# bootphon/abnet3

Hardware: AMD Instinct MI355X
Metric: frame-pairs/sec (Siamese train step: fwd both towers + coscos2 + bwd + Adadelta) (higher is better)
Workload: dtype f16x2; 1 GPU; C2: SiameseNetwork 40->500x2->100 sigmoid, coscos2(avg=False), Adadelta(0.1), 4096 frame pairs per GPU per step, 40-d N(0,1) frames; pairs_per_gpu=4096, global_pairs=4096, parallelism=dp1, graph_replay=False, dp_gradient_buckets=1

## Files before the change

### abnet3_amd/csrc/common.h

```cpp
#pragma once
#include <hip/hip_runtime.h>
#include <stdint.h>
#include <stdio.h>

#include "../../include/abnet3_hip.h"

namespace abn {

void set_error(const char* fmt, ...);

#define ABN_REQUIRE(cond, ...)                      \
    do {                                            \
        if (!(cond)) {                              \
            ::abn::set_error(__VA_ARGS__);          \
            return ABN_E_ARG;                       \
        }                                           \
    } while (0)

#define ABN_CHECK_LAUNCH(what)                                               \
    do {                                                                     \
        hipError_t e_ = hipGetLastError();                                   \
        if (e_ != hipSuccess) {                                              \
            ::abn::set_error("%s: %s", what, hipGetErrorString(e_));         \
            return ABN_E_LAUNCH;                                             \
        }                                                                    \
    } while (0)

struct Switches {
    bool planes;
    bool fused;
    int64_t fused_min_rows;
    bool bn_planes;
    bool bn_persist;
    bool wgrad_xcd;
    bool bf16x3_planes;
    bool bwd_pair;
    int gemm_tile;
    bool dtw_f40, dtw_pc;
    int wgrad_tile128;
    int dtw_wgs_per_cu;
    int wgrad_wgs_heavy, wgrad_wgs_light;
    int64_t wgrad_rows_per_slab;
    bool wide;
    int64_t wide_max_rows;
    int wide_max_groups;
    bool wgrad_step;
    bool dtw_dealt;
    int oneshot_wgs;
    int knn_split;
    int sd_tiles;
};
const Switches& switches();
void reload_switches();

__device__ __forceinline__ bool abn_ticket_publish(double* slot, double value, unsigned* counter, unsigned n_tickets)
{
    __hip_atomic_store(slot, value, __ATOMIC_RELAXED, __HIP_MEMORY_SCOPE_AGENT);
#ifdef ABN_STRICT_FENCES
    const unsigned ticket = __hip_atomic_fetch_add(counter, 1u, __ATOMIC_ACQ_REL, __HIP_MEMORY_SCOPE_AGENT);
#else
    __atomic_signal_fence(__ATOMIC_SEQ_CST);
    __builtin_amdgcn_s_waitcnt(0);
    __atomic_signal_fence(__ATOMIC_SEQ_CST);
    const unsigned ticket = __hip_atomic_fetch_add(counter, 1u, __ATOMIC_RELAXED, __HIP_MEMORY_SCOPE_AGENT);
#endif
    return ticket == n_tickets - 1;
}
__device__ __forceinline__ double abn_ticket_partial(const double* slot)
{
    return __hip_atomic_load(slot, __ATOMIC_RELAXED, __HIP_MEMORY_SCOPE_AGENT);
}

static inline int64_t align_up(int64_t v, int64_t a) { return (v + a - 1) / a * a; }
static inline bool aligned16(const void* p) { return (reinterpret_cast<uintptr_t>(p) & 15) == 0; }

static inline int device_slot()
{
    int dev = 0;
    (void)hipGetDevice(&dev);
    return (dev >= 0 && dev < 16) ? dev : 0;
}
static inline bool first_use_on_device(bool (&seen)[16])
{
    bool& s = seen[device_slot()];
    const bool first = !s;
    s = true;
    return first;
}

}
```

### abnet3_amd/csrc/tower_planes.h

```cpp
#pragma once
#include <type_traits>

#include "gemm_f32.h"

namespace abn {

typedef int v4i __attribute__((ext_vector_type(4)));

constexpr int PL_ROWS = 32;
constexpr int PL_WAVES = 8;
constexpr int PL_NT = 64 * PL_WAVES;
constexpr int PL_MAXW = 512;
constexpr int PL_MAXSTEPS = PL_MAXW / 16;
#ifdef PL_DEPTH_OVERRIDE
constexpr int PL_DEPTH = PL_DEPTH_OVERRIDE;
#else
constexpr int PL_DEPTH = 4;
#endif
constexpr int PL_PART_BYTES = 4 * 16 * 64 * 4;
constexpr int PL_SC_BYTES = PL_WAVES * 64 * 4 + PL_WAVES * 32 * 4;
constexpr int PL_AMAX = 32;

__host__ __device__ inline int pl_steps(int64_t contraction) { return ((int)((contraction + 15) / 16) + PL_DEPTH - 1) / PL_DEPTH * PL_DEPTH; }
__host__ __device__ inline int pl_blocks(int64_t features) { return (int)((features + 31) / 32); }
// ... 930 lines not shown
#pragma unroll
            for (int pl = 0; pl < NP; ++pl) *reinterpret_cast<bf16x8*>(img + ((int64_t)s * NP + pl) * 1024 + lane * 16) = z;
    }
    __syncthreads();
}

template <int NP, bool INFER>
__device__ __forceinline__ void planes_input_stage(const PlanesFwdP& p, char* __restrict__ img, float* __restrict__ part,
                                                   const bf16x8* idf, int wave, int lane, int row0, float& ainv, int row_end = -1)
{
    const int rows_lim = row_end >= 0 ? row_end : p.rows;
    const int r = lane & 31, h = lane >> 5;
    const int D0 = p.dims[0];
    const int steps0 = pl_steps(D0), blocks0 = steps0 / 2;
    const int gr = row0 + r;
    const float* src = nullptr;
    if (gr < rows_lim) src = (p.x2 && gr >= p.rows_call) ? p.x2 + (int64_t)(gr - p.rows_call) * D0 : p.x1 + (int64_t)gr * D0;
    float* const sc = part + PL_PART_BYTES / 4;
    const float* const inv_tab = sc + PL_WAVES * 64 + wave * 32;
    if constexpr (NP == 2) {
        f32x4 v[2][2][2];
        float m = 0.0f;
#pragma unroll
        for (int u = 0; u < 2; ++u) {
            const int kb = wave + PL_WAVES * u;
#pragma unroll
            for (int t2 = 0; t2 < 2; ++t2) {
                const int c0 = 16 * (2 * kb + t2) + 4 * h, c1 = c0 + 8;
                v[u][t2][0] = v[u][t2][1] = f32x4{0.f, 0.f, 0.f, 0.f};
                if (src && kb < blocks0 && c0 < D0) {
                    v[u][t2][0] = *reinterpret_cast<const f32x4*>(src + c0);
                    if (p.x_copy) *reinterpret_cast<f32x4*>(p.x_copy + (int64_t)gr * D0 + c0) = v[u][t2][0];
                }
                if (src && kb < blocks0 && c1 < D0) {
                    v[u][t2][1] = *reinterpret_cast<const f32x4*>(src + c1);
                    if (p.x_copy) *reinterpret_cast<f32x4*>(p.x_copy + (int64_t)gr * D0 + c1) = v[u][t2][1];
                }
                m = fmaxf(m, absmax8(v[u][t2][0], v[u][t2][1]));
            }
        }
        sc[wave * 64 + lane] = m;
        __syncthreads();
        float osc;
        m = row_scales(sc, wave, lane, osc, ainv);
        if (!INFER && p.tp[0] && wave == 0) store_amax_rows(p.amax[0] + (int64_t)blockIdx.x * PL_AMAX, m, 1.0f, lane);
#pragma unroll
        for (int u = 0; u < 2; ++u) {
            const int kb = wave + PL_WAVES * u;
            if (kb < blocks0) {
                Frag<NP> f[2];
#pragma unroll
                for (int t2 = 0; t2 < 2; ++t2) {
                    f[t2] = make_frag<NP>(v[u][t2][0], v[u][t2][1], osc);
                    store_frag<NP>(img + (int64_t)(2 * kb + t2) * (NP * 1024) + lane * 16, f[t2]);
                }
                if (!INFER && p.tp[0] && kb < pl_blocks(D0 + 1))
                    emit_planes<NP>(p.tp[0] + ((int64_t)kb * p.tp_steps + 2 * blockIdx.x) * tile_bytes<NP>(), f, idf, lane,
                                    kb == D0 / 32 ? D0 % 32 : -1, rows_lim - row0, inv_tab);
            }
        }
    } else {
        for (int kb = wave; kb < blocks0; kb += PL_WAVES) {
            Frag<NP> f[2];
#pragma unroll
            for (int t2 = 0; t2 < 2; ++t2) {
                const int s = 2 * kb + t2;
                f32x4 v0 = {0.f, 0.f, 0.f, 0.f}, v1 = v0;
                const int c0 = 16 * s + 4 * h, c1 = c0 + 8;
                if (src && c0 < D0) {
                    v0 = *reinterpret_cast<const f32x4*>(src + c0);
                    if (p.x_copy) *reinterpret_cast<f32x4*>(p.x_copy + (int64_t)gr * D0 + c0) = v0;
                }
                if (src && c1 < D0) {
                    v1 = *reinterpret_cast<const f32x4*>(src + c1);
                    if (p.x_copy) *reinterpret_cast<f32x4*>(p.x_copy + (int64_t)gr * D0 + c1) = v1;
                }
                f[t2] = make_frag<NP>(v0, v1);
                store_frag<NP>(img + (int64_t)s * (NP * 1024) + lane * 16, f[t2]);
            }
            if (!INFER && p.tp[0] && kb < pl_blocks(D0 + 1))
                emit_planes<NP>(p.tp[0] + ((int64_t)kb * p.tp_steps + 2 * blockIdx.x) * tile_bytes<NP>(), f, idf, lane,
                                kb == D0 / 32 ? D0 % 32 : -1, rows_lim - row0);
        }
    }
    if (!INFER && p.tp[0] && pl_blocks(D0 + 1) > blocks0 && wave == PL_WAVES - 1) {
        Frag<NP> z[2] = {};
        emit_planes<NP>(p.tp[0] + ((int64_t)(D0 / 32) * p.tp_steps + 2 * blockIdx.x) * tile_bytes<NP>(), z, idf, lane, 0, rows_lim - row0, inv_tab);
    }
}

template <int NP, int MODE = PL_TRAIN>
__global__ __launch_bounds__(PL_NT) void tower_fwd_planes_kernel(PlanesFwdP p)
{
    constexpr bool INFER = MODE != PL_TRAIN;
    extern __shared__ __attribute__((aligned(16))) char pl_smem[];
    char* const img = pl_smem;
    float* const part = reinterpret_cast<float*>(pl_smem + PL_MAXSTEPS * NP * 1024);
    const int lane = threadIdx.x & 63;
    const int wave = __builtin_amdgcn_readfirstlane(threadIdx.x >> 6);
    const int row0 = blockIdx.x * PL_ROWS;
    bf16x8 idf[2];
    make_identity<NP>(idf, lane);
    PSTAMPF(0);
#ifdef PL_EXP_PRIO
    if ((PL_EXP_PRIO == 1) == (wave >= 4)) __builtin_amdgcn_s_setprio(1);
#endif

    float ainv = 1.0f;
    WeightRing<NP> ring;
    ring_open(ring, p.wbase, p.wbytes);
    constexpr bool STAG = PL_STAGGER && NP <= 2 && (MODE == PL_TRAIN || MODE == PL_INFER);
    Stag st;
    if constexpr (STAG) stag_open(st, pl_smem, NP, threadIdx.x);
    planes_input_stage<NP, INFER>(p, img, part, idf, wave, lane, row0, ainv);
    PSTAMPF(1);
    __syncthreads();

    for (int l = 0; l < p.n_layers; ++l) {
        const int nblk = (p.dims[l + 1] + 31) / 32;
        if constexpr (STAG) {
            char* const cur = st.in();
            const bool out_halves = nblk > PL_WAVES && l + 1 < p.n_layers && (p.dims[l + 2] + 31) / 32 > PL_WAVES;
            if (nblk > PL_WAVES) planes_layer<NP, 2, 1, MODE>(p, l, cur, part, idf, wave, lane, row0, ainv, ring, -1, st, true, out_halves);
            else if (nblk > PL_WAVES / 2 || pl_steps(p.dims[l]) % (2 * PL_DEPTH) != 0) planes_layer<NP, 1, 1, MODE>(p, l, cur, part, idf, wave, lane, row0, ainv, ring);
            else planes_layer<NP, 1, 2, MODE>(p, l, cur, part, idf, wave, lane, row0, ainv, ring);
        } else {
            if (nblk > PL_WAVES) planes_layer<NP, 2, 1, MODE>(p, l, img, part, idf, wave, lane, row0, ainv, ring);
            else if (nblk > PL_WAVES / 2 || pl_steps(p.dims[l]) % (2 * PL_DEPTH) != 0) planes_layer<NP, 1, 1, MODE>(p, l, img, part, idf, wave, lane, row0, ainv, ring);
            else planes_layer<NP, 1, 2, MODE>(p, l, img, part, idf, wave, lane, row0, ainv, ring);
        }
    }
    PSTAMPF(2 + 5 * p.n_layers);
}

struct BnTrainP {
    int l;
    const float* mean;
    const float* invstd;
    const float* z_prev;
    float* a_prev;
    const int* n_valid;
};

template <int NP>
__global__ __launch_bounds__(PL_NT) void bn_fwd_layer_kernel(PlanesFwdP p, BnTrainP q)
{
    extern __shared__ __attribute__((aligned(16))) char pl_smem[];
    char* const img = pl_smem;
    float* const part = reinterpret_cast<float*>(pl_smem + PL_MAXSTEPS * NP * 1024);
    const int lane = threadIdx.x & 63;
    const int wave = __builtin_amdgcn_readfirstlane(threadIdx.x >> 6);
    const int r = lane & 31, h = lane >> 5;
    const int wpc = (p.rows_call + PL_ROWS - 1) / PL_ROWS;
    const int call = blockIdx.x / wpc;
    const int row0 = call * p.rows_call + (blockIdx.x - call * wpc) * PL_ROWS;
    const int row_end = call * p.rows_call + (q.n_valid ? min(max(*q.n_valid, 0), p.rows_call) : p.rows_call);
    const int l = q.l;
    bf16x8 idf[2];
    make_identity<NP>(idf, lane);
    float ainv = 1.0f;
    WeightRing<NP> ring;
    ring_open(ring, p.wbase, p.wbytes);

    if (l == 0) {
        planes_input_stage<NP, false>(p, img, part, idf, wave, lane, row0, ainv, row_end);
    } else {
        const int K = p.dims[l];
        float* const mean_s = part, * const is_s = part + PL_MAXW, * const ga_s = part + 2 * PL_MAXW, * const be_s = part + 3 * PL_MAXW;
        for (int c = threadIdx.x; c < K; c += PL_NT) {
            mean_s[c] = q.mean[(int64_t)call * K + c];
            is_s[c] = q.invstd[(int64_t)call * K + c];
            ga_s[c] = p.bn_w[l - 1][c];
            be_s[c] = p.bn_b[l - 1][c];
        }
        __syncthreads();
        const int steps = pl_steps(K), blocks = steps / 2;
        const int gr = row0 + r;
        const bool row_ok = gr < row_end;
        const float* const zrow = q.z_prev + (int64_t)(row_ok ? gr : row0) * K;
        float* const arow = q.a_prev ? q.a_prev + (int64_t)gr * K : nullptr;
        char* const tp = p.tp[l];
        float* const sc = part + PL_PART_BYTES / 4;
        const float* const inv_tab = sc + PL_WAVES * 64 + wave * 32;
        with_act(p.act[l - 1], [&](auto tag) {
            constexpr int ACT = decltype(tag)::value;
            auto in_step = [&](int s, f32x4* v) {
                v[0] = v[1] = f32x4{0.f, 0.f, 0.f, 0.f};
#pragma unroll
                for (int u = 0; u < 2; ++u) {
                    const int c = 16 * s + 4 * h + 8 * u;
                    if (c < K && row_ok) {
                        const f32x4 z4 = *reinterpret_cast<const f32x4*>(zrow + c);
                        const f32x4 mu = *reinterpret_cast<const f32x4*>(mean_s + c), is = *reinterpret_cast<const f32x4*>(is_s + c);
                        const f32x4 ga = *reinterpret_cast<const f32x4*>(ga_s + c), be = *reinterpret_cast<const f32x4*>(be_s + c);
#pragma unroll
                        for (int e = 0; e < 4; ++e) v[u][e] = act_apply(((z4[e] - mu[e]) * is[e]) * ga[e] + be[e], ACT);
                        if (arow) *reinterpret_cast<f32x4*>(arow + c) = v[u];
                    }
                }
            };
            if constexpr (NP == 2) {
                f32x4 v[2][2][2];
                float m = 0.0f;
#pragma unroll
                for (int u = 0; u < 2; ++u)
#pragma unroll
                    for (int t2 = 0; t2 < 2; ++t2) {
                        const int kb = wave + PL_WAVES * u;
                        v[u][t2][0] = v[u][t2][1] = f32x4{0.f, 0.f, 0.f, 0.f};
                        if (kb < blocks) in_step(2 * kb + t2, v[u][t2]);
                        m = fmaxf(m, absmax8(v[u][t2][0], v[u][t2][1]));
                    }
                sc[wave * 64 + lane] = m;
                __syncthreads();
                float osc;
                m = row_scales(sc, wave, lane, osc, ainv);
                if (tp && wave == 0) store_amax_rows(p.amax[l] + (int64_t)blockIdx.x * PL_AMAX, m, 1.0f, lane);
#pragma unroll
                for (int u = 0; u < 2; ++u) {
                    const int kb = wave + PL_WAVES * u;
                    if (kb < blocks) {
                        Frag<NP> f[2];
#pragma unroll
                        for (int t2 = 0; t2 < 2; ++t2) {
                            f[t2] = make_frag<NP>(v[u][t2][0], v[u][t2][1], osc);
                            store_frag<NP>(img + (int64_t)(2 * kb + t2) * (NP * 1024) + lane * 16, f[t2]);
                        }
                        if (tp && kb < pl_blocks(K + 1))
                            emit_planes<NP>(tp + ((int64_t)kb * p.tp_steps + 2 * blockIdx.x) * tile_bytes<NP>(), f, idf, lane,
                                            kb == K / 32 ? K % 32 : -1, row_end - row0, inv_tab);
                    }
                }
            } else {
                for (int kb = wave; kb < blocks; kb += PL_WAVES) {
                    Frag<NP> f[2];
#pragma unroll
                    for (int t2 = 0; t2 < 2; ++t2) {
                        f32x4 v[2];
                        in_step(2 * kb + t2, v);
                        f[t2] = make_frag<NP>(v[0], v[1]);
                        store_frag<NP>(img + (int64_t)(2 * kb + t2) * (NP * 1024) + lane * 16, f[t2]);
                    }
                    if (tp && kb < pl_blocks(K + 1))
                        emit_planes<NP>(tp + ((int64_t)kb * p.tp_steps + 2 * blockIdx.x) * tile_bytes<NP>(), f, idf, lane,
                                        kb == K / 32 ? K % 32 : -1, row_end - row0);
                }
            }
        });
        if (tp && pl_blocks(K + 1) > blocks && wave == PL_WAVES - 1) {
            Frag<NP> z[2] = {};
            emit_planes<NP>(tp + ((int64_t)(K / 32) * p.tp_steps + 2 * blockIdx.x) * tile_bytes<NP>(), z, idf, lane, 0, row_end - row0, inv_tab);
        }
    }
    __syncthreads();

    const int nblk = (p.dims[l + 1] + 31) / 32;
    if (nblk > PL_WAVES) planes_layer<NP, 2, 1, PL_BN_TRAIN>(p, l, img, part, idf, wave, lane, row0, ainv, ring, row_end);
    else if (nblk > PL_WAVES / 2 || pl_steps(p.dims[l]) % (2 * PL_DEPTH) != 0) planes_layer<NP, 1, 1, PL_BN_TRAIN>(p, l, img, part, idf, wave, lane, row0, ainv, ring, row_end);
    else planes_layer<NP, 1, 2, PL_BN_TRAIN>(p, l, img, part, idf, wave, lane, row0, ainv, ring, row_end);
}

struct PlanesBwdP {
    int n_layers;
    int rows;
    int dims[ABN_MAX_LAYERS + 1];
    int act[ABN_MAX_LAYERS];
    const float* d_out;
    int d_out_is_dz;
    const float* a_top;
    const char* tp[ABN_MAX_LAYERS];
    float* dx;
    const float* mask[ABN_MAX_LAYERS];
    const char* wpt[ABN_MAX_LAYERS];
    const char* wbase;
    int64_t wbytes;
    char* dzp[ABN_MAX_LAYERS];
    float* amax_dz[ABN_MAX_LAYERS];
    int64_t tp_steps;
    const unsigned long long* drop_seed;
    float drop_p;
    int loss_kind;
    int y_dtype;
    const void* y;
    int B;
    double margin, scale;
    double* loss_partial;
    unsigned* loss_counter;
    float* loss_out;
    const int* n_valid;
    double* loss_accum;
#ifdef ABN_STAMPS
    unsigned long long* stamps;
#endif
};
#ifdef ABN_STAMPS
#define DSTAMP(slot) do { if (p.stamps && threadIdx.x == 0) p.stamps[(size_t)blockIdx.x * 64 + (slot)] = __builtin_amdgcn_s_memtime(); } while (0)
#else
#define DSTAMP(slot) do {} while (0)
#endif

template <int NP, int BPW, int KS>
__device__ __forceinline__ void planes_dgrad_layer(const PlanesBwdP& p, int l, char* __restrict__ img,
                                                   float* __restrict__ part, const bf16x8* idf, int wave, int lane, int row0, float& ainv,
                                                   WeightRing<NP>& ring)
{
    const int N = p.dims[l + 1], K = p.dims[l];
    const int nsteps = pl_steps(N), nblk = (K + 31) / 32;
    const int r = lane & 31, h = lane >> 5;
    const WaveShare<BPW, KS> ws(wave, nblk, nsteps);
    const int blk0 = ws.blk0;

    f32x16 acc[BPW];
#pragma unroll
    for (int j = 0; j < BPW; ++j)
#pragma unroll
        for (int q = 0; q < 16; ++q) acc[j][q] = 0.0f;
    float cinv[BPW];
#pragma unroll
    for (int j = 0; j < BPW; ++j) cinv[j] = NP == 2 && ws.active ? packed_inv(p.wpt[l], nblk, nsteps, blk0 + j) * ainv : 1.0f;
    {
        bool chain_next = false;
        int nblk2 = 1, nsteps2 = 0, ioff2 = 0;
        if constexpr (PL_HANDOVER && NP <= 2 && BPW == 2 && KS == 1) {
            if (l - 1 >= (p.dx ? 0 : 1)) {
                nblk2 = (p.dims[l - 1] + 31) / 32;
                nsteps2 = pl_steps(K);
                ioff2 = (int)(p.wpt[l - 1] - p.wbase);
                chain_next = nblk2 > PL_WAVES;
            }
        }
        if (!ws.active) ring.filled = false;
        const int ioff = (int)(p.wpt[l] - p.wbase);
        int wv[BPW], dnext[BPW];
#pragma unroll
        for (int j = 0; j < BPW; ++j) {
            const int blk = blk0 + j < nblk ? blk0 + j : nblk - 1;
            const int o = ioff + (blk * nsteps + ws.s_first) * (NP * 1024);
            const int blk2 = blk0 + j < nblk2 ? blk0 + j : nblk2 - 1;
            wv[j] = o + lane * 16;
            dnext[j] = ioff2 + blk2 * nsteps2 * (NP * 1024) - o;
        }
        if (ws.active) ring_kloop<NP, BPW>(acc, ring, wv, dnext, chain_next, img, ws.s_first, ws.my_steps, lane);
    }
    DSTAMP(4 + 4 * (p.n_layers - 1 - l));

    const float* __restrict__ mask = l >= 1 ? p.mask[l - 1] : nullptr;
    const DropGen drop = make_drop(l >= 1 && !mask ? p.drop_seed : nullptr, p.drop_p, l - 1);
    const bool masked = mask || drop.on;
    const int gr = row0 + r;
    const bool row_ok = gr < p.rows;
    const int grc = row_ok ? gr : p.rows - 1;
    f32x4 av[BPW][4], mv[BPW][4];
    if (ws.active && ws.khalf == 0 && l >= 1) {
        const int row_off = tgather_row_offset<NP>(r);
#pragma unroll
        for (int j = 0; j < BPW; ++j) {
            const int blk = blk0 + j < nblk ? blk0 + j : nblk - 1;
            const char* tile = p.tp[l] + ((int64_t)blk * p.tp_steps + 2 * blockIdx.x) * tile_bytes<NP>();
#pragma unroll
            for (int g = 0; g < 4; ++g) {
#pragma unroll
                for (int e = 0; e < 4; ++e) av[j][g][e] = tgather<NP>(tile, row_off, 8 * g + 4 * h + e);
                const int k = 32 * (blk0 + j) + 4 * h + 8 * g;
                if (mask) mv[j][g] = *reinterpret_cast<const f32x4*>(mask + (int64_t)grc * K + (k < K ? k : K - 4));
                else if (drop.on) mv[j][g] = drop4(drop, gr, k);
            }
        }
    }
    auto finish = [&]() {
        if constexpr (NP == 2) {
#pragma unroll
            for (int j = 0; j < BPW; ++j)
#pragma unroll
                for (int q = 0; q < 16; ++q) acc[j][q] *= cinv[j];
        }
        if (l == 0) return;
        with_act(p.act[l - 1], [&](auto tag) {
            constexpr int ACT = decltype(tag)::value;
#pragma unroll
            for (int j = 0; j < BPW; ++j)
#pragma unroll
                for (int g = 0; g < 4; ++g) {
                    const bool live = 32 * (blk0 + j) + 4 * h + 8 * g < K;
#pragma unroll
                    for (int e = 0; e < 4; ++e) {
                        float v = acc[j][4 * g + e] * act_grad(av[j][g][e], ACT);
                        if (masked) v *= mv[j][g][e];
                        acc[j][4 * g + e] = live ? v : 0.0f;
                    }
                }
        });
    };
    float* const sc = part + PL_PART_BYTES / 4;
    const bool rescale = NP == 2 && l >= 1;
    auto park_max = [&]() {
        float m = 0.0f;
        if (ws.active && ws.khalf == 0) {
#pragma unroll
            for (int j = 0; j < BPW; ++j)
#pragma unroll
                for (int q = 0; q < 16; ++q) m = fmaxf(m, fabsf(acc[j][q]));
        }
        sc[wave * 64 + lane] = m;
    };
    if (KS == 1) {
        if (ws.active) finish();
        if (rescale) park_max();
    } else if (ws.active && ws.khalf == 1) {
#pragma unroll
        for (int q = 0; q < 16; ++q) part[((wave & 3) * 16 + q) * 64 + lane] = acc[0][q];
    }
    DSTAMP(5 + 4 * (p.n_layers - 1 - l));
    __syncthreads();
    DSTAMP(6 + 4 * (p.n_layers - 1 - l));
    if (KS == 2 && ws.active && ws.khalf == 0) {
#pragma unroll
        for (int q = 0; q < 16; ++q) acc[0][q] += part[(wave * 16 + q) * 64 + lane];
        finish();
    }
    float osc = 1.0f;
    if (rescale) {
        if (KS == 2) { park_max(); __syncthreads(); }
        float oinv;
        const float m = row_scales(sc, wave, lane, osc, oinv);
        ainv = oinv;
        if (wave == 0) store_amax_rows(p.amax_dz[l - 1] + (int64_t)blockIdx.x * PL_AMAX, m, 0.0f, lane);
    }
    const float* const inv_tab = sc + PL_WAVES * 64 + wave * 32;
    if (ws.active && ws.khalf == 0) {
#pragma unroll
        for (int j = 0; j < BPW; ++j) {
            const int blk = blk0 + j;
            if (blk < nblk) {
                Frag<NP> f[2];
#pragma unroll
                for (int t2 = 0; t2 < 2; ++t2) {
                    const f32x4 v0 = {acc[j][8 * t2], acc[j][8 * t2 + 1], acc[j][8 * t2 + 2], acc[j][8 * t2 + 3]};
                    const f32x4 v1 = {acc[j][8 * t2 + 4], acc[j][8 * t2 + 5], acc[j][8 * t2 + 6], acc[j][8 * t2 + 7]};
                    if (l == 0) {
                        const int k = 32 * blk + 16 * t2 + 4 * h;
                        if (row_ok && k < K) *reinterpret_cast<f32x4*>(p.dx + (int64_t)gr * K + k) = v0;
                        if (row_ok && k + 8 < K) *reinterpret_cast<f32x4*>(p.dx + (int64_t)gr * K + k + 8) = v1;
                    } else {
                        f[t2] = make_frag<NP>(v0, v1, osc);
                        store_frag<NP>(img + (int64_t)(2 * blk + t2) * (NP * 1024) + lane * 16, f[t2]);
                    }
                }
                if (l >= 1) emit_planes<NP>(p.dzp[l - 1] + ((int64_t)blk * p.tp_steps + 2 * blockIdx.x) * tile_bytes<NP>(), f, idf, lane, -1, 0, inv_tab);
            }
        }
    }
    if (l - 1 >= 1 || (l == 1 && p.dx)) {
        const int next_steps = pl_steps(K);
        const bf16x8 z = {};
        for (int s = 2 * nblk + wave; s < next_steps; s += PL_WAVES)
#pragma unroll
            for (int pl = 0; pl < NP; ++pl) *reinterpret_cast<bf16x8*>(img + ((int64_t)s * NP + pl) * 1024 + lane * 16) = z;
    }
    __syncthreads();
    DSTAMP(7 + 4 * (p.n_layers - 1 - l));
}

template <int NP>
__global__ __launch_bounds__(PL_NT) void tower_dgrad_planes_kernel(PlanesBwdP p)
{
    extern __shared__ __attribute__((aligned(16))) char pl_smem[];
    char* const img = pl_smem;
    float* const part = reinterpret_cast<float*>(pl_smem + PL_MAXSTEPS * NP * 1024);
    const int lane = threadIdx.x & 63;
    const int wave = __builtin_amdgcn_readfirstlane(threadIdx.x >> 6);
    const int r = lane & 31, h = lane >> 5;
    const int row0 = blockIdx.x * PL_ROWS;
    const int top = p.n_layers - 1;
    const int NT = p.dims[top + 1];
    bf16x8 idf[2];
    make_identity<NP>(idf, lane);
#ifdef PL_EXP_PRIO
    if ((PL_EXP_PRIO == 1) == (wave >= 4)) __builtin_amdgcn_s_setprio(1);
#endif
    DSTAMP(0);

    double* const coef = reinterpret_cast<double*>(part);
    double* const term_s = coef + 64;
    int* const is_last_s = reinterpret_cast<int*>(term_s + 32);
    const bool with_loss = p.loss_kind >= 0;
    if (with_loss) {
        const int B = p.B;
        const int Bv = p.n_valid ? *p.n_valid : B;
        const double lscale = p.n_valid && p.scale != 1.0 ? 1.0 / (double)(Bv > 0 ? Bv : 1) : p.scale;
#pragma unroll
        for (int it = 0; it < 2; ++it) {
            const int lr = 4 * wave + 2 * it + (lane >> 5), l = lane & 31;
            const int g = row0 + lr;
            double inv = 0.0, kself = 0.0, term = 0.0;
            const int tower = g < p.rows && g >= B ? 1 : 0, pi_ = g < p.rows ? g - tower * B : 0;
            const bool ok = g < p.rows && pi_ < Bv;
            const float* a = p.a_top + (int64_t)pi_ * NT;
            const float* b = p.a_top + (int64_t)(B + pi_) * NT;
            double dot = 0.0, s11 = 0.0, s22 = 0.0;
            for (int c = l; c < NT / 4; c += 32) {
                const float4 u = reinterpret_cast<const float4*>(a)[c];
                const float4 v = reinterpret_cast<const float4*>(b)[c];
                dot += (double)u.x * v.x + (double)u.y * v.y + (double)u.z * v.z + (double)u.w * v.w;
                s11 += (double)u.x * u.x + (double)u.y * u.y + (double)u.z * u.z + (double)u.w * u.w;
                s22 += (double)v.x * v.x + (double)v.y * v.y + (double)v.z * v.z + (double)v.w * v.w;
            }
#pragma unroll
            for (int o = 16; o >= 1; o >>= 1) {
                dot += __shfl_xor(dot, o, 64);
                s11 += __shfl_xor(s11, o, 64);
                s22 += __shfl_xor(s22, o, 64);
            }
            if (ok) {
                constexpr double EPS = 1e-6;
                const double n1 = sqrt(s11), n2 = sqrt(s22);
                const double c1 = n1 > EPS ? n1 : EPS, c2 = n2 > EPS ? n2 : EPS;
                const double cs = dot / (c1 * c2);
                double v = 0.0;
                switch (p.y_dtype) {
                    case ABN_Y_I8: v = ((const int8_t*)p.y)[pi_]; break;
                    case ABN_Y_I32: v = ((const int32_t*)p.y)[pi_]; break;
                    case ABN_Y_I64: v = (double)((const int64_t*)p.y)[pi_]; break;
                    case ABN_Y_F32: v = ((const float*)p.y)[pi_]; break;
                    default: v = ((const double*)p.y)[pi_]; break;
                }
                const int code = v == 1.0 ? 1 : (v == -1.0 ? -1 : 0);
                double dcos;
                if (p.loss_kind == ABN_LOSS_COSCOS2) {
                    if (code == 1) { term = (1.0 - cs) * 0.5; dcos = -0.5; }
                    else if (code == -1) { term = cs * cs; dcos = 2.0 * cs; }
                    else { term = cs; dcos = 1.0; }
                } else {
                    if (code == 1) { term = 1.0 - cs; dcos = -1.0; }
                    else if (code == -1) { const double hh = cs - p.margin; term = hh > 0.0 ? hh : 0.0; dcos = hh >= 0.0 ? 1.0 : 0.0; }
                    else { term = cs; dcos = 1.0; }
                }
                dcos *= lscale;
                inv = dcos / (c1 * c2);
                const double k1 = n1 > 0.0 ? dcos * cs / (c1 * n1) : 0.0;
                const double k2 = n2 > 0.0 ? dcos * cs / (c2 * n2) : 0.0;
                kself = tower ? k2 : k1;
                if (tower) term = 0.0;
            }
            if (l == 0) { coef[2 * lr] = inv; coef[2 * lr + 1] = kself; term_s[lr] = term; }
        }
        __syncthreads();
        if (threadIdx.x == 0) {
            double sum = 0.0;
            for (int i = 0; i < 32; ++i) sum += term_s[i];
            *is_last_s = abn_ticket_publish(&p.loss_partial[blockIdx.x], sum, p.loss_counter, gridDim.x);
        }
        __syncthreads();
        if (*is_last_s && wave == 0) {
            double sum = 0.0;
            for (int i = lane; i < (int)gridDim.x; i += 64) sum += abn_ticket_partial(&p.loss_partial[i]);
#pragma unroll
            for (int o = 32; o >= 1; o >>= 1) sum += __shfl_xor(sum, o, 64);
            if (lane == 0) {
                const float lv = (float)(sum * lscale);
                *p.loss_out = lv;
                if (p.loss_accum) *p.loss_accum += (double)lv;
                __hip_atomic_store(p.loss_counter, 0u, __ATOMIC_RELAXED, __HIP_MEMORY_SCOPE_AGENT);
            }
        }
    }

    DSTAMP(1);
    const int steps_t = pl_steps(NT), blocks_t = steps_t / 2;
    const int gr = row0 + r;
    const bool row_ok = gr < p.rows;
    const float* __restrict__ mask = p.mask[top];
    const DropGen drop_top = make_drop(mask ? nullptr : p.drop_seed, p.drop_p, top);
    const int my_tower = gr >= p.B ? 1 : 0;
    const float* const self_row = p.a_top + (int64_t)(row_ok ? gr : 0) * NT;
    const float* const partner_row = p.a_top + (int64_t)(row_ok && with_loss ? (my_tower ? gr - p.B : gr + p.B) : 0) * NT;
    const double my_inv = with_loss ? coef[2 * r] : 0.0, my_k = with_loss ? coef[2 * r + 1] : 0.0;
    auto top_step = [&](int s, f32x4* v) {
        v[0] = v[1] = f32x4{0.f, 0.f, 0.f, 0.f};
#pragma unroll
        for (int u = 0; u < 2; ++u) {
            const int c = 16 * s + 4 * h + 8 * u;
            if (row_ok && c < NT) {
                if (with_loss) {
                    const f32x4 es = *reinterpret_cast<const f32x4*>(self_row + c);
                    const f32x4 ep = *reinterpret_cast<const f32x4*>(partner_row + c);
#pragma unroll
                    for (int e = 0; e < 4; ++e) {
                        float o = (float)(ep[e] * my_inv - es[e] * my_k);
                        if (p.act[top] != ACT_NONE) o *= act_grad(es[e], p.act[top]);
                        v[u][e] = o;
                    }
                    if (mask || drop_top.on) {
                        const f32x4 m = mask ? *reinterpret_cast<const f32x4*>(mask + (int64_t)gr * NT + c) : drop4(drop_top, gr, c);
#pragma unroll
                        for (int e = 0; e < 4; ++e) v[u][e] *= m[e];
                    }
                } else {
                    v[u] = *reinterpret_cast<const f32x4*>(p.d_out + (int64_t)gr * NT + c);
                    if (!p.d_out_is_dz) {
                        const f32x4 a = *reinterpret_cast<const f32x4*>(p.a_top + (int64_t)gr * NT + c);
#pragma unroll
                        for (int e = 0; e < 4; ++e) v[u][e] *= act_grad(a[e], p.act[top]);
                        if (mask || drop_top.on) {
                            const f32x4 m = mask ? *reinterpret_cast<const f32x4*>(mask + (int64_t)gr * NT + c) : drop4(drop_top, gr, c);
#pragma unroll
                            for (int e = 0; e < 4; ++e) v[u][e] *= m[e];
                        }
                    }
                }
            }
        }
    };
    float ainv = 1.0f;
    if constexpr (NP == 2) {
        float* const sc = part + PL_PART_BYTES / 4;
        f32x4 v[2][2][2];
        float m = 0.0f;
#pragma unroll
        for (int u = 0; u < 2; ++u)
#pragma unroll
            for (int t2 = 0; t2 < 2; ++t2) {
                const int kb = wave + PL_WAVES * u;
                v[u][t2][0] = v[u][t2][1] = f32x4{0.f, 0.f, 0.f, 0.f};
                if (kb < blocks_t) top_step(2 * kb + t2, v[u][t2]);
                m = fmaxf(m, absmax8(v[u][t2][0], v[u][t2][1]));
            }
        sc[wave * 64 + lane] = m;
        __syncthreads();
        float osc;
        m = row_scales(sc, wave, lane, osc, ainv);
        if (wave == 0) store_amax_rows(p.amax_dz[top] + (int64_t)blockIdx.x * PL_AMAX, m, 0.0f, lane);
#pragma unroll
        for (int u = 0; u < 2; ++u) {
            const int kb = wave + PL_WAVES * u;
            if (kb < blocks_t) {
                Frag<NP> f[2];
#pragma unroll
                for (int t2 = 0; t2 < 2; ++t2) {
                    f[t2] = make_frag<NP>(v[u][t2][0], v[u][t2][1], osc);
                    store_frag<NP>(img + (int64_t)(2 * kb + t2) * (NP * 1024) + lane * 16, f[t2]);
                }
                if (kb < pl_blocks(NT))
                    emit_planes<NP>(p.dzp[top] + ((int64_t)kb * p.tp_steps + 2 * blockIdx.x) * tile_bytes<NP>(), f, idf, lane, -1, 0,
                                    sc + PL_WAVES * 64 + wave * 32);
            }
        }
    } else {
        for (int kb = wave; kb < blocks_t; kb += PL_WAVES) {
            Frag<NP> f[2];
#pragma unroll
            for (int t2 = 0; t2 < 2; ++t2) {
                f32x4 v[2];
                top_step(2 * kb + t2, v);
                f[t2] = make_frag<NP>(v[0], v[1]);
                store_frag<NP>(img + (int64_t)(2 * kb + t2) * (NP * 1024) + lane * 16, f[t2]);
            }
            if (kb < pl_blocks(NT))
                emit_planes<NP>(p.dzp[top] + ((int64_t)kb * p.tp_steps + 2 * blockIdx.x) * tile_bytes<NP>(), f, idf, lane, -1, 0);
        }
    }
    __syncthreads();
    DSTAMP(2);

    WeightRing<NP> ring;
    ring_open(ring, p.wbase, p.wbytes);
    for (int l = top; l >= (p.dx ? 0 : 1); --l) {
        const int nblk = (p.dims[l] + 31) / 32;
        if (nblk > PL_WAVES) planes_dgrad_layer<NP, 2, 1>(p, l, img, part, idf, wave, lane, row0, ainv, ring);
        else if (nblk > PL_WAVES / 2 || pl_steps(p.dims[l + 1]) % (2 * PL_DEPTH) != 0) planes_dgrad_layer<NP, 1, 1>(p, l, img, part, idf, wave, lane, row0, ainv, ring);
        else planes_dgrad_layer<NP, 1, 2>(p, l, img, part, idf, wave, lane, row0, ainv, ring);
    }
}

struct BnBwdP {
    int l, rows, rows_call;
    float n_stat;
    const float* n_stat_dev;
    int N, K;
    int act_l, act_prev;
    const float* da;
    const float* z;
    const float* mean;
    const float* invstd;
    const float* gamma;
    const float* beta;
    const float* s1;
    const float* s2;
    const float* mask;
    const unsigned long long* drop_seed;
    float drop_p;
    char* dzp;
    float* amax_dz;
    int64_t tp_steps;
    const char* wpt;
    float* da_prev;
    const float* z_prev;
    const float* mean_prev;
    const float* invstd_prev;
    const float* gamma_prev;
    const float* beta_prev;
    float* part_out;
    const int* n_valid;
};

template <int NP, int BPW, int KS>
__device__ __forceinline__ void bn_dgrad_product(const BnBwdP& q, char* __restrict__ img, float* __restrict__ part, int wave,
                                                 int lane, int row0, int row_end, int call, float ainv)
{
    const int N = q.N, K = q.K;
    const int nsteps = pl_steps(N), nblk = (K + 31) / 32;
    const int r = lane & 31, h = lane >> 5;
    const WaveShare<BPW, KS> ws(wave, nblk, nsteps);
    const int blk0 = ws.blk0;
    f32x16 acc[BPW];
#pragma unroll
    for (int j = 0; j < BPW; ++j)
#pragma unroll
        for (int x = 0; x < 16; ++x) acc[j][x] = 0.0f;
    if (ws.active) planes_kloop<NP, BPW>(acc, q.wpt, nblk, nsteps, img, blk0, ws.s_first, ws.my_steps, lane);
    if (KS == 2 && ws.active && ws.khalf == 1) {
#pragma unroll
        for (int x = 0; x < 16; ++x) part[((wave & 3) * 16 + x) * 64 + lane] = acc[0][x];
    }
    if (KS == 2) __syncthreads();
    if (!(ws.active && ws.khalf == 0)) return;
    if (KS == 2) {
#pragma unroll
        for (int x = 0; x < 16; ++x) acc[0][x] += part[(wave * 16 + x) * 64 + lane];
    }
    if constexpr (NP == 2) {
#pragma unroll
        for (int j = 0; j < BPW; ++j) {
            const float cinv = packed_inv(q.wpt, nblk, nsteps, blk0 + j) * ainv;
#pragma unroll
            for (int x = 0; x < 16; ++x) acc[j][x] *= cinv;
        }
    }
    const int gr = row0 + r;
    const bool row_ok = gr < row_end;
    const int grc = row_ok ? gr : row0;
    float* const orow = q.da_prev + (int64_t)grc * K;
    float* const pw = q.l >= 1 ? q.part_out + (int64_t)blockIdx.x * (2 * PL_MAXW) : nullptr;
    with_act(q.act_prev, [&](auto tag) {
        constexpr int ACT = decltype(tag)::value;
#pragma unroll
        for (int j = 0; j < BPW; ++j)
#pragma unroll
            for (int g = 0; g < 4; ++g) {
                const int n = 32 * (blk0 + j) + 8 * g + 4 * h;
                const bool live = n < K;
                const f32x4 d4 = {acc[j][4 * g], acc[j][4 * g + 1], acc[j][4 * g + 2], acc[j][4 * g + 3]};
                if (live && row_ok) *reinterpret_cast<f32x4*>(orow + n) = d4;
                if (q.l >= 1) {
                    const int nc = live ? n : K - 4;
                    const f32x4 z4 = *reinterpret_cast<const f32x4*>(q.z_prev + (int64_t)grc * K + nc);
                    const f32x4 mu = *reinterpret_cast<const f32x4*>(q.mean_prev + (int64_t)call * K + nc);
                    const f32x4 is = *reinterpret_cast<const f32x4*>(q.invstd_prev + (int64_t)call * K + nc);
                    f32x4 xh;
#pragma unroll
                    for (int e = 0; e < 4; ++e) xh[e] = (z4[e] - mu[e]) * is[e];
                    const f32x4 ga = *reinterpret_cast<const f32x4*>(q.gamma_prev + nc), be = *reinterpret_cast<const f32x4*>(q.beta_prev + nc);
                    f32x4 sd, sq;
#pragma unroll
                    for (int e = 0; e < 4; ++e) {
                        const float a = act_apply(xh[e] * ga[e] + be[e], ACT);
                        const float dy = live && row_ok ? d4[e] * act_grad(a, ACT) : 0.0f;
                        sd[e] = dy;
                        sq[e] = dy * xh[e];
                    }
                    half_wave_sum4(sd);
                    half_wave_sum4(sq);
                    if (r == 16 && live) {
                        *reinterpret_cast<f32x4*>(pw + n) = sd;
                        *reinterpret_cast<f32x4*>(pw + PL_MAXW + n) = sq;
                    }
                }
            }
    });
}

template <int NP>
__global__ __launch_bounds__(PL_NT) void bn_bwd_layer_kernel(BnBwdP q)
{
    extern __shared__ __attribute__((aligned(16))) char pl_smem[];
    char* const img = pl_smem;
    float* const part = reinterpret_cast<float*>(pl_smem + PL_MAXSTEPS * NP * 1024);
    const int lane = threadIdx.x & 63;
    const int wave = __builtin_amdgcn_readfirstlane(threadIdx.x >> 6);
    const int r = lane & 31, h = lane >> 5;
    const int wpc = (q.rows_call + PL_ROWS - 1) / PL_ROWS;
    const int call = blockIdx.x / wpc;
    const int row0 = call * q.rows_call + (blockIdx.x - call * wpc) * PL_ROWS;
    const int nv = q.n_valid ? min(max(*q.n_valid, 0), q.rows_call) : q.rows_call;
    const int row_end = call * q.rows_call + nv;
    const int N = q.N;
    bf16x8 idf[2];
    make_identity<NP>(idf, lane);

    const float nf = q.n_valid ? (float)(nv > 0 ? nv : 1) : (q.n_stat_dev ? q.n_stat_dev[call] : q.n_stat);
    float* const k_s = part, * const ga_s = part + PL_MAXW, * const be_s = part + 2 * PL_MAXW, * const s1_s = part + 3 * PL_MAXW,
               * const s2_s = part + 4 * PL_MAXW, * const mu_s = part + 5 * PL_MAXW, * const is_s = part + 6 * PL_MAXW;
    for (int c = threadIdx.x; c < N; c += PL_NT) {
        const float ga = q.gamma[c];
        k_s[c] = ga * q.invstd[(int64_t)call * N + c] / nf;
        mu_s[c] = q.mean[(int64_t)call * N + c];
        is_s[c] = q.invstd[(int64_t)call * N + c];
        ga_s[c] = ga;
        be_s[c] = q.beta[c];
        s1_s[c] = q.s1[(int64_t)call * N + c];
        s2_s[c] = q.s2[(int64_t)call * N + c];
    }
    __syncthreads();
    const int steps = pl_steps(N), blocks = steps / 2;
    const int gr = row0 + r;
    const bool row_ok = gr < row_end;
    const int grc = row_ok ? gr : row0;
    const float* const drow = q.da + (int64_t)grc * N;
    const float* const zrow = q.z + (int64_t)grc * N;
    const float* const mrow = q.mask ? q.mask + (int64_t)grc * N : nullptr;
    const DropGen drop = make_drop(q.mask ? nullptr : q.drop_seed, q.drop_p, q.l);
    float* const sc = part + PL_PART_BYTES / 4;
    float ainv = 1.0f;
    with_act(q.act_l, [&](auto tag) {
        constexpr int ACT = decltype(tag)::value;
        auto dz_step = [&](int s, f32x4* v) {
            v[0] = v[1] = f32x4{0.f, 0.f, 0.f, 0.f};
#pragma unroll
            for (int u = 0; u < 2; ++u) {
                const int c = 16 * s + 4 * h + 8 * u;
                if (c < N && row_ok) {
                    const f32x4 d4 = *reinterpret_cast<const f32x4*>(drow + c), z4 = *reinterpret_cast<const f32x4*>(zrow + c);
                    const f32x4 mu = *reinterpret_cast<const f32x4*>(mu_s + c), is = *reinterpret_cast<const f32x4*>(is_s + c);
                    f32x4 xh;
#pragma unroll
                    for (int e = 0; e < 4; ++e) xh[e] = (z4[e] - mu[e]) * is[e];
                    const f32x4 k4 = *reinterpret_cast<const f32x4*>(k_s + c), ga = *reinterpret_cast<const f32x4*>(ga_s + c);
                    const f32x4 be = *reinterpret_cast<const f32x4*>(be_s + c);
                    const f32x4 a1 = *reinterpret_cast<const f32x4*>(s1_s + c), a2 = *reinterpret_cast<const f32x4*>(s2_s + c);
                    f32x4 m4 = {1.f, 1.f, 1.f, 1.f};
                    if (mrow) m4 = *reinterpret_cast<const f32x4*>(mrow + c);
                    else if (drop.on) m4 = drop4(drop, gr, c);
#pragma unroll
                    for (int e = 0; e < 4; ++e) {
                        const float a = act_apply(xh[e] * ga[e] + be[e], ACT);
                        const float dy = d4[e] * act_grad(a, ACT);
                        v[u][e] = k4[e] * (nf * dy - a1[e] - xh[e] * a2[e]) * m4[e];
                    }
                }
            }
        };
        if constexpr (NP == 2) {
            f32x4 v[2][2][2];
            float m = 0.0f;
#pragma unroll
            for (int u = 0; u < 2; ++u)
#pragma unroll
                for (int t2 = 0; t2 < 2; ++t2) {
                    const int kb = wave + PL_WAVES * u;
                    v[u][t2][0] = v[u][t2][1] = f32x4{0.f, 0.f, 0.f, 0.f};
                    if (kb < blocks) dz_step(2 * kb + t2, v[u][t2]);
                    m = fmaxf(m, absmax8(v[u][t2][0], v[u][t2][1]));
                }
            sc[wave * 64 + lane] = m;
            __syncthreads();
            float osc;
            m = row_scales(sc, wave, lane, osc, ainv);
            if (wave == 0) store_amax_rows(q.amax_dz + (int64_t)blockIdx.x * PL_AMAX, m, 0.0f, lane);
#pragma unroll
            for (int u = 0; u < 2; ++u) {
                const int kb = wave + PL_WAVES * u;
                if (kb < blocks) {
                    Frag<NP> f[2];
#pragma unroll
                    for (int t2 = 0; t2 < 2; ++t2) {
                        f[t2] = make_frag<NP>(v[u][t2][0], v[u][t2][1], osc);
                        store_frag<NP>(img + (int64_t)(2 * kb + t2) * (NP * 1024) + lane * 16, f[t2]);
                    }
                    if (kb < pl_blocks(N))
                        emit_planes<NP>(q.dzp + ((int64_t)kb * q.tp_steps + 2 * blockIdx.x) * tile_bytes<NP>(), f, idf, lane, -1, 0,
                                        sc + PL_WAVES * 64 + wave * 32);
                }
            }
        } else {
            for (int kb = wave; kb < blocks; kb += PL_WAVES) {
                Frag<NP> f[2];
#pragma unroll
                for (int t2 = 0; t2 < 2; ++t2) {
                    f32x4 v[2];
                    dz_step(2 * kb + t2, v);
                    f[t2] = make_frag<NP>(v[0], v[1]);
                    store_frag<NP>(img + (int64_t)(2 * kb + t2) * (NP * 1024) + lane * 16, f[t2]);
                }
                if (kb < pl_blocks(N))
                    emit_planes<NP>(q.dzp + ((int64_t)kb * q.tp_steps + 2 * blockIdx.x) * tile_bytes<NP>(), f, idf, lane, -1, 0);
            }
        }
    });
    __syncthreads();
    if (!q.wpt) return;

    const int nblk = (q.K + 31) / 32;
    if (nblk > PL_WAVES) bn_dgrad_product<NP, 2, 1>(q, img, part, wave, lane, row0, row_end, call, ainv);
    else if (nblk > PL_WAVES / 2 || pl_steps(N) % (2 * PL_DEPTH) != 0) bn_dgrad_product<NP, 1, 1>(q, img, part, wave, lane, row0, row_end, call, ainv);
    else bn_dgrad_product<NP, 1, 2>(q, img, part, wave, lane, row0, row_end, call, ainv);
}

template <int NP> constexpr int wg_stages() { return NP >= 2 ? 4 : 6; }
constexpr int WG_REG_DEPTH = 4;
constexpr int WG_MAX_BLOCKS = 12;
struct WgradLayer {
    const char* dzp;
    const char* ap;
    int N, K;
    int nblk, kblk;
    int shape;
    int tiles_n, tiles_k;
    int splits;
    int first_wg;
    int64_t slab_off;
    const float* amax_dz;
    const float* amax_a;
};
struct WgradP {
    int n_layers;
    WgradLayer L[ABN_MAX_LAYERS];
    float* slabs;
    int64_t slab_stride;
    int64_t tp_steps;
    int xcd_groups;
#ifdef ABN_STAMPS
    unsigned long long* stamps;
#endif
};

__host__ __device__ inline int wgrad_group_count(int g0, int splits, int x, int* first)
{
    *first = g0 + ((x - g0) & 7);
    return *first < g0 + splits ? (g0 + splits - 1 - *first) / 8 + 1 : 0;
}
static inline int wgrad_slots(const WgradP& p, int x)
{
    int slots = 0, g0 = 0, first;
    for (int i = 0; i < p.n_layers; ++i) {
        slots += wgrad_group_count(g0, p.L[i].splits, x, &first) * p.L[i].tiles_n * p.L[i].tiles_k;
        g0 += p.L[i].splits;
    }
    return slots;
}
static inline void wgrad_shape(int nblk, int kblk, int* shape, int* bn, int* bk, bool small_tiles = false)
{
    if (small_tiles) { *shape = 3; *bn = 4; *bk = 4; return; }
    if (kblk <= 2) { *shape = 1; *bn = 8; *bk = 2; }
    else if (nblk <= 4) { *shape = 2; *bn = 4; *bk = 8; }
    else { *shape = 0; *bn = 8; *bk = 4; }
}

template <int NP>
constexpr size_t wgrad_lds_bytes() { return (size_t)wg_stages<NP>() * WG_MAX_BLOCKS * (NP * 1024) + (NP == 2 ? 128 : 0); }

template <int NP, int TN, int TK, int WN, int WK>
__device__ __forceinline__ void wgrad_tile(const WgradP& p, const WgradLayer& L, char* __restrict__ smem, int nb0, int kb0,
                                           int s_begin, int s_end, int split, int wave, int lane)
{
    static_assert(WN * WK == PL_WAVES, "eight waves");
    constexpr int BN = WN * TN, BK_ = WK * TK, NB = BN + BK_;
    constexpr int PER_WAVE = (NB + PL_WAVES - 1) / PL_WAVES;
    constexpr int FR = tile_bytes<NP>();
    constexpr int DI = FR / 1024;
    constexpr int STAGE = NB * FR;
    constexpr int WG_STAGES = wg_stages<NP>();
    static_assert(NB <= WG_MAX_BLOCKS, "LDS stage");
    constexpr int PSTAGE = NB * NP * 1024;
    const int wn = wave % WN, wk = wave / WN;
    const char* src[PER_WAVE];
// ... 321 lines not shown
```

Before: 25.38 million frame-pairs/s.

## Defer loss ticket draw into top dgrad layer to hide atomic latency

Splits the loss-reduction ticket into a post (store the partial) and a separate draw (atomic counter increment). The draw is moved into the first dgrad layer after its loads are issued, and the final loss reduction runs after the dgrad loop. This removes a block-wide barrier and the wait on the atomic from the critical path between loss and backward. Mask and dropout loads are also split from the tile gathers, and the activation scale is applied at finish time. The risk is in memory ordering: without the explicit waitcnt, the partial store may not be visible before the counter increment.

```diff
diff --git a/abnet3_amd/csrc/common.h b/abnet3_amd/csrc/common.h
--- a/abnet3_amd/csrc/common.h
+++ b/abnet3_amd/csrc/common.h
@@ -53,9 +53,23 @@
 const Switches& switches();
 void reload_switches();
 
-__device__ __forceinline__ bool abn_ticket_publish(double* slot, double value, unsigned* counter, unsigned n_tickets)
+__device__ __forceinline__ void abn_ticket_post(double* slot, double value)
 {
     __hip_atomic_store(slot, value, __ATOMIC_RELAXED, __HIP_MEMORY_SCOPE_AGENT);
+    __atomic_signal_fence(__ATOMIC_SEQ_CST);
+}
+__device__ __forceinline__ bool abn_ticket_draw_acked(unsigned* counter, unsigned n_tickets)
+{
+    __atomic_signal_fence(__ATOMIC_SEQ_CST);
+#ifdef ABN_STRICT_FENCES
+    const unsigned ticket = __hip_atomic_fetch_add(counter, 1u, __ATOMIC_ACQ_REL, __HIP_MEMORY_SCOPE_AGENT);
+#else
+    const unsigned ticket = __hip_atomic_fetch_add(counter, 1u, __ATOMIC_RELAXED, __HIP_MEMORY_SCOPE_AGENT);
+#endif
+    return ticket == n_tickets - 1;
+}
+__device__ __forceinline__ bool abn_ticket_draw(unsigned* counter, unsigned n_tickets)
+{
 #ifdef ABN_STRICT_FENCES
     const unsigned ticket = __hip_atomic_fetch_add(counter, 1u, __ATOMIC_ACQ_REL, __HIP_MEMORY_SCOPE_AGENT);
 #else
@@ -65,6 +79,11 @@
     const unsigned ticket = __hip_atomic_fetch_add(counter, 1u, __ATOMIC_RELAXED, __HIP_MEMORY_SCOPE_AGENT);
 #endif
     return ticket == n_tickets - 1;
+}
+__device__ __forceinline__ bool abn_ticket_publish(double* slot, double value, unsigned* counter, unsigned n_tickets)
+{
+    abn_ticket_post(slot, value);
+    return abn_ticket_draw(counter, n_tickets);
 }
 __device__ __forceinline__ double abn_ticket_partial(const double* slot)
 {
diff --git a/abnet3_amd/csrc/tower_planes.h b/abnet3_amd/csrc/tower_planes.h
--- a/abnet3_amd/csrc/tower_planes.h
+++ b/abnet3_amd/csrc/tower_planes.h
@@ -1256,7 +1256,7 @@
 template <int NP, int BPW, int KS>
 __device__ __forceinline__ void planes_dgrad_layer(const PlanesBwdP& p, int l, char* __restrict__ img,
                                                    float* __restrict__ part, const bf16x8* idf, int wave, int lane, int row0, float& ainv,
-                                                   WeightRing<NP>& ring)
+                                                   WeightRing<NP>& ring, bool draw, bool& is_last)
 {
     const int N = p.dims[l + 1], K = p.dims[l];
     const int nsteps = pl_steps(N), nblk = (K + 31) / 32;
@@ -1269,9 +1269,10 @@
     for (int j = 0; j < BPW; ++j)
 #pragma unroll
         for (int q = 0; q < 16; ++q) acc[j][q] = 0.0f;
-    float cinv[BPW];
-#pragma unroll
-    for (int j = 0; j < BPW; ++j) cinv[j] = NP == 2 && ws.active ? packed_inv(p.wpt[l], nblk, nsteps, blk0 + j) * ainv : 1.0f;
+    float winv[BPW];
+    const float ainv_in = ainv;
+#pragma unroll
+    for (int j = 0; j < BPW; ++j) winv[j] = NP == 2 && ws.active ? packed_inv(p.wpt[l], nblk, nsteps, blk0 + j) : 1.0f;
     {
         bool chain_next = false;
         int nblk2 = 1, nsteps2 = 0, ioff2 = 0;
@@ -1312,21 +1313,37 @@
             const int blk = blk0 + j < nblk ? blk0 + j : nblk - 1;
             const char* tile = p.tp[l] + ((int64_t)blk * p.tp_steps + 2 * blockIdx.x) * tile_bytes<NP>();
 #pragma unroll
-            for (int g = 0; g < 4; ++g) {
+            for (int g = 0; g < 4; ++g)
 #pragma unroll
                 for (int e = 0; e < 4; ++e) av[j][g][e] = tgather<NP>(tile, row_off, 8 * g + 4 * h + e);
-                const int k = 32 * (blk0 + j) + 4 * h + 8 * g;
-                if (mask) mv[j][g] = *reinterpret_cast<const f32x4*>(mask + (int64_t)grc * K + (k < K ? k : K - 4));
-                else if (drop.on) mv[j][g] = drop4(drop, gr, k);
-            }
-        }
-    }
+        }
+        if (masked) {
+#pragma unroll
+            for (int j = 0; j < BPW; ++j)
+#pragma unroll
+                for (int g = 0; g < 4; ++g) {
+                    const int k = 32 * (blk0 + j) + 4 * h + 8 * g;
+                    if (mask) mv[j][g] = *reinterpret_cast<const f32x4*>(mask + (int64_t)grc * K + (k < K ? k : K - 4));
+                    else mv[j][g] = drop4(drop, gr, k);
+                }
+        }
+#ifdef ABN_STAMPS
+#pragma unroll
+        for (int j = 0; j < BPW; ++j)
+#pragma unroll
+            for (int g = 0; g < 4; ++g) asm volatile("" : "+v"(av[j][g]));
+#endif
+    }
+    DSTAMP(32 + (p.n_layers - 1 - l));
+    if (draw && threadIdx.x == 0) is_last = abn_ticket_draw_acked(p.loss_counter, gridDim.x);
     auto finish = [&]() {
         if constexpr (NP == 2) {
 #pragma unroll
-            for (int j = 0; j < BPW; ++j)
-#pragma unroll
-                for (int q = 0; q < 16; ++q) acc[j][q] *= cinv[j];
+            for (int j = 0; j < BPW; ++j) {
+                const float cinv = winv[j] * ainv_in;
+#pragma unroll
+                for (int q = 0; q < 16; ++q) acc[j][q] *= cinv;
+            }
         }
         if (l == 0) return;
         with_act(p.act[l - 1], [&](auto tag) {
@@ -1436,8 +1453,8 @@
 
     double* const coef = reinterpret_cast<double*>(part);
     double* const term_s = coef + 64;
-    int* const is_last_s = reinterpret_cast<int*>(term_s + 32);
     const bool with_loss = p.loss_kind >= 0;
+    bool is_last = false;
     if (with_loss) {
         const int B = p.B;
         const int Bv = p.n_valid ? *p.n_valid : B;
@@ -1499,23 +1516,11 @@
             if (l == 0) { coef[2 * lr] = inv; coef[2 * lr + 1] = kself; term_s[lr] = term; }
         }
         __syncthreads();
+        DSTAMP(3);
         if (threadIdx.x == 0) {
             double sum = 0.0;
             for (int i = 0; i < 32; ++i) sum += term_s[i];
-            *is_last_s = abn_ticket_publish(&p.loss_partial[blockIdx.x], sum, p.loss_counter, gridDim.x);
-        }
-        __syncthreads();
-        if (*is_last_s && wave == 0) {
-            double sum = 0.0;
-            for (int i = lane; i < (int)gridDim.x; i += 64) sum += abn_ticket_partial(&p.loss_partial[i]);
-#pragma unroll
-            for (int o = 32; o >= 1; o >>= 1) sum += __shfl_xor(sum, o, 64);
-            if (lane == 0) {
-                const float lv = (float)(sum * lscale);
-                *p.loss_out = lv;
-                if (p.loss_accum) *p.loss_accum += (double)lv;
-                __hip_atomic_store(p.loss_counter, 0u, __ATOMIC_RELAXED, __HIP_MEMORY_SCOPE_AGENT);
-            }
+            abn_ticket_post(&p.loss_partial[blockIdx.x], sum);
         }
     }
 
@@ -1618,12 +1623,33 @@
 
     WeightRing<NP> ring;
     ring_open(ring, p.wbase, p.wbytes);
-    for (int l = top; l >= (p.dx ? 0 : 1); --l) {
+    const int l_last = p.dx ? 0 : 1;
+    for (int l = top; l >= l_last; --l) {
+        const bool draw = with_loss && l == top;
         const int nblk = (p.dims[l] + 31) / 32;
-        if (nblk > PL_WAVES) planes_dgrad_layer<NP, 2, 1>(p, l, img, part, idf, wave, lane, row0, ainv, ring);
-        else if (nblk > PL_WAVES / 2 || pl_steps(p.dims[l + 1]) % (2 * PL_DEPTH) != 0) planes_dgrad_layer<NP, 1, 1>(p, l, img, part, idf, wave, lane, row0, ainv, ring);
-        else planes_dgrad_layer<NP, 1, 2>(p, l, img, part, idf, wave, lane, row0, ainv, ring);
-    }
+        if (nblk > PL_WAVES) planes_dgrad_layer<NP, 2, 1>(p, l, img, part, idf, wave, lane, row0, ainv, ring, draw, is_last);
+        else if (nblk > PL_WAVES / 2 || pl_steps(p.dims[l + 1]) % (2 * PL_DEPTH) != 0) planes_dgrad_layer<NP, 1, 1>(p, l, img, part, idf, wave, lane, row0, ainv, ring, draw, is_last);
+        else planes_dgrad_layer<NP, 1, 2>(p, l, img, part, idf, wave, lane, row0, ainv, ring, draw, is_last);
+    }
+    DSTAMP(40);
+    if (with_loss && wave == 0) {
+        if (top < l_last && threadIdx.x == 0) is_last = abn_ticket_draw(p.loss_counter, gridDim.x);
+        if (__builtin_amdgcn_readfirstlane((int)is_last)) {
+            const int Bv = p.n_valid ? *p.n_valid : p.B;
+            const double lscale = p.n_valid && p.scale != 1.0 ? 1.0 / (double)(Bv > 0 ? Bv : 1) : p.scale;
+            double sum = 0.0;
+            for (int i = lane; i < (int)gridDim.x; i += 64) sum += abn_ticket_partial(&p.loss_partial[i]);
+#pragma unroll
+            for (int o = 32; o >= 1; o >>= 1) sum += __shfl_xor(sum, o, 64);
+            if (lane == 0) {
+                const float lv = (float)(sum * lscale);
+                *p.loss_out = lv;
+                if (p.loss_accum) *p.loss_accum += (double)lv;
+                __hip_atomic_store(p.loss_counter, 0u, __ATOMIC_RELAXED, __HIP_MEMORY_SCOPE_AGENT);
+            }
+        }
+    }
+    DSTAMP(41);
 }
 
 struct BnBwdP {
```

Result: no change. 25.52 million frame-pairs/s (median of 6 runs) (+0.6%).
